# imazen/codec-eval

Hardware: AMD Instinct MI355X
Metric: metric MP/s (SSIMULACRA2+DSSIM+Butteraugli) at 1/2/4/8 GPU; HBM-roofline % (higher is better)
Workload: dtype f32

## Files before the change

### codec-eval_amd/__init__.py

```python
from __future__ import annotations

import ctypes as C
import os
from dataclasses import dataclass
from typing import Iterable, List, Optional, Sequence, Tuple

import numpy as np

os.environ.setdefault("GPU_MAX_HW_QUEUES", "16")

_HERE = os.path.dirname(os.path.abspath(__file__))
LIB_PATH = os.environ.get("CE_METRICS_LIB") or os.path.join(_HERE, "libce_metrics_hip.so")
INCLUDE_DIR = os.path.join(os.path.dirname(_HERE), "include")

CE_OK, CE_ERR_DIM_MISMATCH, CE_ERR_BAD_LENGTH, CE_ERR_TOO_SMALL, CE_ERR_BACKEND, CE_ERR_INVALID_ARG = range(6)
METRIC_DSSIM, METRIC_SSIMULACRA2, METRIC_BUTTERAUGLI, METRIC_PSNR = 1, 2, 4, 8
FLAG_XYB_ROUNDTRIP = 1
FLAG_BUTTERAUGLI_DIFFMAP = 1 << 1
FLAG_SSIMULACRA2_MAPS = 1 << 2
PIXEL_RGB8, PIXEL_RGBA8, PIXEL_RGB16_10BIT, PIXEL_RGBA16_10BIT = 0, 1, 2, 3
BATCH_REFERENCES, BATCH_TESTS = 0, 1
DEFAULT_INTENSITY_TARGET = 80.0
DSSIM_MAX_LEVELS = 5
SSIM2_MAX_SCALES = 6
# ... 678 lines not shown
        self.ctx._check(lib().ce_batch_set_test_lut(self._h, pair_index, ref_index, a.ctypes.data, a.nbytes, fmt, table._h if table else None))

    def bind_pair(self, pair_index: int, ref_index: int):
        self.ctx._check(lib().ce_batch_bind_pair(self._h, pair_index, ref_index))

    @property
    def reference_slab(self) -> int:
        return int(lib().ce_batch_reference_slab(self._h))

    @property
    def test_slab(self) -> int:
        return int(lib().ce_batch_test_slab(self._h))

    def run(self, n_pairs: int, config: MetricConfig, intensity_target: float = DEFAULT_INTENSITY_TARGET,
            butteraugli_diffmap: bool = False, ssimulacra2_maps: bool = False) -> List[CeScores]:
        out = (CeScores * n_pairs)()
        flags = config.flags | (FLAG_BUTTERAUGLI_DIFFMAP if butteraugli_diffmap else 0) | (FLAG_SSIMULACRA2_MAPS if ssimulacra2_maps else 0)
        self.ctx._check(lib().ce_batch_run(self._h, n_pairs, config.mask, flags, intensity_target, out))
        return list(out)

    def launch(self, n_pairs: int, config: MetricConfig, intensity_target: float = DEFAULT_INTENSITY_TARGET,
               butteraugli_diffmap: bool = False, ssimulacra2_maps: bool = False):
        flags = config.flags | (FLAG_BUTTERAUGLI_DIFFMAP if butteraugli_diffmap else 0) | (FLAG_SSIMULACRA2_MAPS if ssimulacra2_maps else 0)
        self.ctx._check(lib().ce_batch_launch(self._h, n_pairs, config.mask, flags, intensity_target))

    def collect(self, n_pairs: int) -> List[CeScores]:
        out = (CeScores * n_pairs)()
        self.ctx._check(lib().ce_batch_collect(self._h, n_pairs, out))
        return list(out)

    def butteraugli_pnorm3(self, n_pairs: int) -> np.ndarray:
        out = np.zeros(n_pairs, np.float64)
        self.ctx._check(lib().ce_batch_butteraugli_pnorm3(self._h, n_pairs, out.ctypes.data_as(_dp)))
        return out

    def butteraugli_diffmaps(self, first: int, count: int, block: int = 1) -> np.ndarray:
        return _read_diffmaps(self.ctx, lib().ce_batch_butteraugli_diffmap, self._h, self.width, self.height, first, count, block)

    def dssim_ssim_maps(self, level: int, first: int, count: int, block: int = 1):
        return _read_ssim_maps(self.ctx, lib().ce_batch_dssim_ssim_maps, self._h, self.width, self.height, level, first, count, block)

    def ssimulacra2_maps(self, scale: int, channel: int, kind: int, first: int, count: int, block: int = 1, maps: bool = True):
        return _read_ssim2_maps(self.ctx, lib().ce_batch_ssimulacra2_maps, self._h, self.width, self.height, scale, channel, kind,
                                first, count, block, maps)

    def image_heuristics(self, first: int, count: int, tests: bool = False) -> List[ImageHeuristics]:
        out = (CeImageHeuristics * max(count, 1))()
        self.ctx._check(lib().ce_batch_image_heuristics(self._h, BATCH_TESTS if tests else BATCH_REFERENCES, first, count, out))
        return [ImageHeuristics.from_c(out[i]) for i in range(count)]

    def debug_limit_scales(self, n: int):
        self.ctx._check(lib().ce_debug_ssim2_limit_scales(self._h, n))

    def debug_planes(self, scale: int, which: int, channel: int = 0) -> np.ndarray:
        nplanes = 5 if which == 4 else 3
        buf = np.empty(nplanes * self.width * self.height, np.float32)
        w, h = C.c_uint32(), C.c_uint32()
        self.ctx._check(lib().ce_debug_ssim2_planes(self._h, scale, which, channel, buf.ctypes.data, buf.size,
                                                     C.byref(w), C.byref(h)))
        return buf[: nplanes * w.value * h.value].reshape(nplanes, h.value, w.value).copy()

    def debug_dssim_walk_rows(self, rows: int):
        self.ctx._check(lib().ce_debug_dssim_walk_rows(self._h, rows))

    def debug_averages(self, pair_index: int) -> np.ndarray:
        avg = np.zeros((6, 3, 6), np.float64)
        ns = C.c_int()
        self.ctx._check(lib().ce_debug_ssim2_averages(self._h, pair_index, avg.ctypes.data_as(_dp), C.byref(ns)))
        return avg[: ns.value].copy()


class ReferenceHandle:

    def __init__(self, ctx: Context, reference, width: int, height: int, xyb_roundtrip: bool = False,
                 butteraugli_diffmap: bool = False, ssimulacra2_maps: bool = False):
        self.ctx, self.width, self.height = ctx, width, height
        r = _buf(reference)
        self._h = C.c_void_p()
        flags = ((FLAG_XYB_ROUNDTRIP if xyb_roundtrip else 0) | (FLAG_BUTTERAUGLI_DIFFMAP if butteraugli_diffmap else 0) |
                 (FLAG_SSIMULACRA2_MAPS if ssimulacra2_maps else 0))
        ctx._check(lib().ce_ref_create(ctx._h, r.ctypes.data, r.size, width, height, flags, C.byref(self._h)))

    def compare(self, test, config: MetricConfig = None, intensity_target: float = DEFAULT_INTENSITY_TARGET) -> MetricResult:
        config = config or MetricConfig.ssimulacra2_only()
        t = _buf(test)
        s = CeScores()
        self.ctx._check(lib().ce_ref_compare(self._h, t.ctypes.data, t.size, config.mask, intensity_target, C.byref(s)))
        return MetricResult.from_c(s)

    def compare_many(self, tests, config: MetricConfig = None, intensity_target: float = DEFAULT_INTENSITY_TARGET):
        config = config or MetricConfig.ssimulacra2_only()
        bufs = [_buf(t) for t in tests]
        n = len(bufs)
        if n == 0:
            return []
        ptrs = (C.c_void_p * n)(*[b.ctypes.data for b in bufs])
        lens = (_sz * n)(*[b.size for b in bufs])
        out = (CeScores * n)()
        self.ctx._check(lib().ce_ref_compare_many(self._h, ptrs, lens, n, config.mask, intensity_target, out))
        res = []
        for s in out:
            res.append(MetricResult.from_c(s) if s.status == 0 else _error_obj(s.status, self.ctx._err()))
        return res

    def butteraugli_diffmaps(self, first: int, count: int, block: int = 1) -> np.ndarray:
        return _read_diffmaps(self.ctx, lib().ce_ref_butteraugli_diffmap, self._h, self.width, self.height, first, count, block)

    def dssim_ssim_maps(self, level: int, first: int, count: int, block: int = 1):
# ... 104 lines not shown
```

### codec-eval_amd/csrc/ce_api.cpp

```cpp
#include <algorithm>
#include <atomic>
#include <condition_variable>
#include <functional>
#include <mutex>
#include <thread>
#include <cmath>
#include <cstdlib>
#include <cstring>
#include <new>

#include "ce_internal.h"

namespace {

thread_local std::string g_err_noctx;

int fail(ce_ctx *ctx, int code, const std::string &msg)
{
    if (ctx) ctx->err = msg; else g_err_noctx = msg;
    return code;
}

int bad_length(ce_ctx *ctx, size_t want, size_t got)
{
// ... 1595 lines not shown
    ctx->prof_filter = substring ? substring : "";
    return CE_OK;
}

int ce_prof_reset(ce_ctx *ctx)
{
    if (!ctx) return CE_ERR_INVALID_ARG;
    prof_drain(ctx);
    ctx->stats.clear();
    return CE_OK;
}

int ce_prof_count(ce_ctx *ctx)
{
    if (!ctx) return 0;
    prof_drain(ctx);
    return (int)ctx->stats.size();
}

int ce_prof_get(ce_ctx *ctx, int index, const char **name, uint64_t *launches, double *total_ms)
{
    if (!ctx || index < 0 || index >= (int)ctx->stats.size()) return CE_ERR_INVALID_ARG;
    prof_drain(ctx);
    if (name) *name = ctx->stats[index].name.c_str();
    if (launches) *launches = ctx->stats[index].launches;
    if (total_ms) *total_ms = ctx->stats[index].total_ms;
    return CE_OK;
}

int ce_timer_start(ce_ctx *ctx)
{
    if (!ctx) return CE_ERR_INVALID_ARG;
    CE_HIP(ctx, hipSetDevice(ctx->device));
    CE_HIP(ctx, hipEventRecord(ctx->t0, ctx->stream));
    return CE_OK;
}

int ce_timer_stop(ce_ctx *ctx, double *elapsed_ms)
{
    if (!ctx || !elapsed_ms) return CE_ERR_INVALID_ARG;
    CE_HIP(ctx, hipSetDevice(ctx->device));
    CE_HIP(ctx, hipEventRecord(ctx->t1, ctx->stream));
    CE_HIP(ctx, hipEventSynchronize(ctx->t1));
    float ms = 0.f;
    CE_HIP(ctx, hipEventElapsedTime(&ms, ctx->t0, ctx->t1));
    *elapsed_ms = ms;
    return CE_OK;
}


int ce_debug_ssim2_planes(ce_batch *b, int scale, int which, int channel, float *out, size_t out_floats,
                          uint32_t *w_out, uint32_t *h_out)
{
    if (!b || !out || !b->ssim2_ready || scale < 0 || scale >= b->n_scales) return CE_ERR_INVALID_ARG;
    ce_ctx *ctx = b->ctx;
    const ce_scale_dims &d = b->sd[scale];
    const int nplanes = which == 4 ? CE_SSIM2_STREAMS : 3;
    if (out_floats < (size_t)nplanes * d.w * d.h) return CE_ERR_INVALID_ARG;
    const uint32_t ref_slot = b->h_pair_ref[0], test_slot = b->max_refs;
    const float *src = nullptr;
    switch (which) {
        case 0:
        case 1:
            if (scale == 0) return CE_ERR_INVALID_ARG;
            src = b->d_lin[scale] + (size_t)(which == 0 ? ref_slot : test_slot) * 3 * d.plane;
            break;
        case 2: src = b->d_xyb[scale] + (size_t)ref_slot * 3 * d.plane; break;
        case 3: src = b->d_xyb[scale] + (size_t)test_slot * 3 * d.plane; break;
        case 4:
            if (channel < 0 || channel > 2) return CE_ERR_INVALID_ARG;
            src = b->d_hbuf[scale] + (size_t)channel * CE_SSIM2_STREAMS * d.hplane;
            break;
        default: return CE_ERR_INVALID_ARG;
    }
    CE_HIP(ctx, hipSetDevice(ctx->device));
    CE_HIP(ctx, hipStreamSynchronize(ctx->stream));
    const size_t spl = which == 4 ? d.hplane : d.plane, spitch = which == 4 ? d.hpitch : d.pitch;
    for (int p = 0; p < nplanes; p++)
        CE_HIP(ctx, hipMemcpy2D(out + (size_t)p * d.w * d.h, (size_t)d.w * sizeof(float), src + (size_t)p * spl,
                                spitch * sizeof(float), (size_t)d.w * sizeof(float), d.h, hipMemcpyDeviceToHost));
    if (w_out) *w_out = d.w;
    if (h_out) *h_out = d.h;
    return CE_OK;
}

int ce_debug_ssim2_limit_scales(ce_batch *b, int max_scales)
{
    if (!b || max_scales < 1 || max_scales > CE_MAX_SCALES) return CE_ERR_INVALID_ARG;
    b->debug_max_scales = max_scales;
    return CE_OK;
}

int ce_debug_dssim_walk_rows(ce_batch *b, uint32_t rows)
{
    if (!b || (rows != 0 && (rows < 2 || rows > 64 || (rows & (rows - 1)) != 0))) return CE_ERR_INVALID_ARG;
    b->debug_ds_rows = rows;
    return CE_OK;
}

int ce_debug_ssim2_averages(ce_batch *b, uint32_t pair_index, double *avg, int *n_scales)
{
    if (!b || !avg || !b->ssim2_ready || pair_index >= b->max_pairs) return CE_ERR_INVALID_ARG;
    ce_ctx *ctx = b->ctx;
    CE_HIP(ctx, hipSetDevice(ctx->device));
    CE_HIP(ctx, hipStreamSynchronize(ctx->stream));
    CE_HIP(ctx, hipMemcpy(avg, b->d_avg + (size_t)pair_index * CE_MAX_SCALES * 18, sizeof(double) * CE_MAX_SCALES * 18,
                          hipMemcpyDeviceToHost));
    if (n_scales) *n_scales = b->n_scales;
    return CE_OK;
}

int ce_debug_ssim2_occupancy(int which) { return ce_ssim2_occupancy(which); }

int ce_debug_div_sweep(ce_ctx *ctx, uint64_t seed, uint64_t count, uint64_t *mismatches)
{
    if (!ctx || count == 0) return CE_ERR_INVALID_ARG;
    CE_HIP(ctx, hipSetDevice(ctx->device));
    return ce_butteraugli_div_sweep(ctx, seed, count, mismatches);
}

int ce_debug_calibrate_traffic(ce_ctx *ctx, size_t bytes)
{
    if (!ctx) return CE_ERR_INVALID_ARG;
    CE_HIP(ctx, hipSetDevice(ctx->device));
// ... 12 lines not shown
```

### codec-eval_amd/csrc/ce_plan.h

```cpp
#pragma once

#include <algorithm>
#include <cstdint>
#include <map>
#include <vector>

inline constexpr uint32_t ce_plan_ring_slots = 3;
inline constexpr size_t ce_plan_none = ~(size_t)0;

struct ce_plan_inputs {
    size_t budget;
    size_t per_pair;
    uint32_t pooled_pairs;
    size_t forced_chunks;
    size_t ramp;
};

struct ce_plan_chunk {
    uint32_t slot;
    uint32_t max_pairs;
    size_t collect_first;
    std::vector<std::vector<size_t>> refs;
};

inline void ce_plan_bucket(const std::vector<size_t> &items, const std::vector<const void *> &refs, const ce_plan_inputs &in,
                           uint32_t &ring, std::vector<ce_plan_chunk> &plan)
{
    std::map<const void *, size_t> group_of;
    std::vector<std::vector<size_t>> groups;
    for (size_t j = 0; j < items.size(); j++) {
        const size_t g = group_of.emplace(refs[j], groups.size()).first->second;
        if (g == groups.size()) groups.emplace_back();
        groups[g].push_back(items[j]);
    }
    const size_t n = items.size();
    const size_t n_chunks = in.forced_chunks ? std::min<size_t>(in.forced_chunks, std::max<size_t>(1, n))
                                             : std::min<size_t>(ce_plan_ring_slots, std::max<size_t>(1, n / 64));
    size_t target = std::min((n + n_chunks - 1) / n_chunks, std::max<size_t>(1, in.budget / std::max<size_t>(in.per_pair, 1)));
    if (in.pooled_pairs < target && (size_t)in.pooled_pairs * 4 >= target * 3) target = in.pooled_pairs;
    std::vector<std::vector<size_t>> split;
    for (auto &g : groups)
        for (size_t o = 0; o < g.size(); o += target) split.emplace_back(g.begin() + o, g.begin() + std::min(g.size(), o + target));
    const bool several = n > target;
    size_t limit = (several && in.ramp && ring == 0) ? std::min(in.ramp, target) : target;
    const size_t bucket_begin = plan.size();
    for (size_t g0 = 0, g1 = 0; g0 < split.size(); g0 = g1) {
        size_t count = 0;
        while (g1 < split.size() && (count == 0 || count + split[g1].size() <= limit)) count += split[g1++].size();
        limit = std::min(target, limit * 2);
        ce_plan_chunk c{ring++ % ce_plan_ring_slots, (uint32_t)(several ? std::max(count, target) : count), ce_plan_none,
                        std::vector<std::vector<size_t>>(split.begin() + g0, split.begin() + g1)};
        for (size_t p = bucket_begin; p < plan.size(); p++)
            if (plan[p].slot == c.slot) c.collect_first = p;
        plan.push_back(std::move(c));
    }
}

struct ce_plan_entry {
    uint32_t tile, pair;
};

struct ce_xcd_keys {
    uint32_t channels;
    uint32_t keys_per_channel;
    uint32_t tiles_per_key;
    uint32_t round_to = 1;
};

inline bool operator==(const ce_xcd_keys &a, const ce_xcd_keys &b)
{
    return a.channels == b.channels && a.keys_per_channel == b.keys_per_channel && a.tiles_per_key == b.tiles_per_key &&
           a.round_to == b.round_to;
}

inline std::vector<ce_plan_entry> ce_plan_xcd_list(const uint32_t *pair_ref, uint32_t n_pairs, uint32_t n_refs, const ce_xcd_keys &k)
{
    std::vector<std::vector<uint32_t>> pairs_of(n_refs);
    for (uint32_t p = 0; p < n_pairs; p++) pairs_of[pair_ref[p]].push_back(p);
    std::vector<ce_plan_entry> cls[8];
    uint32_t key = 0;
    for (const auto &pairs : pairs_of) {
        if (pairs.empty()) continue;
        for (uint32_t c = 0; c < k.channels; c++)
            for (uint32_t j = 0; j < k.keys_per_channel; j++, key++)
                for (uint32_t sub = 0; sub < k.tiles_per_key; sub++)
                    for (uint32_t p : pairs) cls[key & 7].push_back({(j * k.tiles_per_key + sub) | c << 16, p});
    }
    size_t len = 0;
    for (const auto &v : cls) len = std::max(len, v.size());
    len = (len + k.round_to - 1) / k.round_to * k.round_to;
    std::vector<ce_plan_entry> list(len * 8, ce_plan_entry{~0u, 0u});
    for (uint32_t x = 0; x < 8; x++)
        for (size_t i = 0; i < cls[x].size(); i++) list[i * 8 + x] = cls[x][i];
    return list;
}

inline uint32_t ce_plan_dssim_levels(uint32_t w, uint32_t h, uint32_t max_levels, uint32_t *level_w, uint32_t *level_h)
{
    if (w == 0 || h == 0) return 0;
    uint32_t n = 0;
    while (n < max_levels) {
        level_w[n] = w;
        level_h[n] = h;
        n++;
        if (w < 8 || h < 8) break;
        w /= 2;
        h /= 2;
    }
    return n;
}

inline uint32_t ce_plan_ssim2_scales(uint32_t w, uint32_t h, uint32_t max_scales, uint32_t *scale_w, uint32_t *scale_h)
{
    uint32_t n = 0;
    for (uint32_t s = 0; s < max_scales; s++) {
        if (w < 8 || h < 8) break;
        if (s > 0) {
            w = w / 2 + (w & 1);
            h = h / 2 + (h & 1);
        }
        scale_w[n] = w;
        scale_h[n] = h;
        n++;
    }
    return n;
}
```

### codec-eval_amd/csrc/ssim2.hip

```cpp
#include <algorithm>
#include <cstdlib>

#include "ce_internal.h"

namespace {

struct rg_consts {
    float mul_in[3];
    float mul_prev[3];
};

constexpr int kColsPerBlock = 64;

constexpr int kTailLevels = CE_MAX_SCALES - 1;
struct lvl_table {
    uint32_t n, first_level;
    uint32_t blk_end[kTailLevels];
    uint32_t w[kTailLevels], h[kTailLevels], pitch[kTailLevels];
    size_t plane[kTailLevels];
    const float *xyb[kTailLevels];
    float *hbuf[kTailLevels];
};

__device__ __forceinline__ uint32_t slot_of(uint32_t z, uint32_t n_refs_used, uint32_t max_refs)
// ... 124 lines not shown
            }
            sum[0] += r;
            sum[1] += g;
            sum[2] += bl;
            linear_to_xyb_positive(r, g, bl, cbrt_bias, X[dx], Y[dx], B[dx]);
        }
        if (yr < h) {
            const size_t o = (size_t)y * pitch + 2 * qx;
            if (2 * qx + 1 < w) {
                *reinterpret_cast<float2 *>(xo + o) = make_float2(X[0], X[1]);
                *reinterpret_cast<float2 *>(xo + o + plane) = make_float2(Y[0], Y[1]);
                *reinterpret_cast<float2 *>(xo + o + 2 * plane) = make_float2(B[0], B[1]);
            } else {
                xo[o] = X[0];
                xo[o + plane] = Y[0];
                xo[o + 2 * plane] = B[0];
            }
        }
    }
    if (has_next) {
        float *lo = lin_out + (size_t)slot * 3 * oplane + (size_t)qy * opitch + qx;
        lo[0] = sum[0] * 0.25f;
        lo[oplane] = sum[1] * 0.25f;
        lo[2 * oplane] = sum[2] * 0.25f;
    }
}

__device__ __forceinline__ float rg_step(float sum, float (&prev)[3], float (&prev2)[3], const rg_consts &rg)
{
    float o[3];
#pragma unroll
    for (int k = 0; k < 3; k++) {
        float v = sum * rg.mul_in[k];
        v = __builtin_fmaf(-1.0f, prev2[k], v);
        prev2[k] = prev[k];
        v = __builtin_fmaf(rg.mul_prev[k], prev[k], v);
        prev[k] = v;
        o[k] = v;
    }
    return o[0] + o[1] + o[2];
}

__device__ __forceinline__ void lds_barrier()
{
    asm volatile("" ::: "memory");
    __builtin_amdgcn_s_waitcnt(0xC07F);
    __builtin_amdgcn_s_barrier();
    asm volatile("" ::: "memory");
}

#ifndef CE_HB_ROWS
#define CE_HB_ROWS 32
#endif
constexpr int HB_ROWS = CE_HB_ROWS, HB_CW = 32, HB_LD = HB_ROWS + 1, HB_THREADS = 256;
constexpr int HB_LOADS = 2 * HB_ROWS * 8;
constexpr int HB_LSLOTS = (HB_LOADS + 63) / 64;
static_assert(HB_ROWS * CE_SSIM2_STREAMS <= HB_THREADS, "one task per thread");
constexpr int HB_HALF = HB_CW * HB_LD;
constexpr int HB_STORES = CE_SSIM2_STREAMS * HB_ROWS * (HB_CW / 4);

typedef float hb_f2 __attribute__((ext_vector_type(2)));

struct hblur_state {
    hb_f2 p01, q01;
    float p2, q2;
    float d[10];
};

__device__ __forceinline__ void hblur_chunk(const float *__restrict__ p_cur, const float *__restrict__ q_cur, bool plain,
                                            float *__restrict__ so, hblur_state &st, const rg_consts &rg)
{
    const hb_f2 n01 = {rg.mul_in[0], rg.mul_in[1]}, d01 = {rg.mul_prev[0], rg.mul_prev[1]};
#pragma unroll
    for (int half = 0; half < 2; half++) {
        float in[HB_CW / 2];
#pragma unroll
        for (int i = 0; i < HB_CW / 2; i++) in[i] = p_cur[(half * (HB_CW / 2) + i) * HB_LD];
#pragma unroll
        for (int i = 0; i < HB_CW / 2; i++) {
            const float q = q_cur[(half * (HB_CW / 2) + i) * HB_LD];
            in[i] = in[i] * (plain ? 1.0f : q);
        }
#pragma unroll
        for (int i = 0; i < HB_CW / 2; i++) {
            const int e = half * (HB_CW / 2) + i;
            const float sum = st.d[e % 10] + in[i];
            st.d[e % 10] = in[i];
            hb_f2 v01 = hb_f2{sum, sum} * n01;
            v01 = v01 - st.q01;
            st.q01 = st.p01;
            v01 = __builtin_elementwise_fma(d01, st.p01, v01);
            st.p01 = v01;
            float v2 = sum * rg.mul_in[2];
            v2 = v2 - st.q2;
            st.q2 = st.p2;
            v2 = __builtin_fmaf(rg.mul_prev[2], st.p2, v2);
            st.p2 = v2;
            so[e * HB_LD] = v01.x + v01.y + v2;
        }
    }
    float t[10];
#pragma unroll
    for (int j = 0; j < 10; j++) t[j] = st.d[(j + HB_CW) % 10];
#pragma unroll
    for (int j = 0; j < 10; j++) st.d[j] = t[j];
}

template <int LEVEL>
__global__ __launch_bounds__(HB_THREADS) void k_ssim2_hblur_lds(const float *__restrict__ xyb,
                                                                const uint32_t *__restrict__ pair_ref,
                                                                float *__restrict__ hbuf, uint32_t w, uint32_t h,
                                                                uint32_t pitch, size_t plane, uint32_t max_refs,
                                                                rg_consts rg, lvl_table tab, const uint2 *__restrict__ work,
                                                                const uint32_t *__restrict__ pair_first)
{
    __shared__ float s_in[2][2 * HB_HALF];
    __shared__ float s_out[CE_SSIM2_STREAMS * HB_HALF];
    const uint32_t tid = threadIdx.x, lane = tid & 63, wv = tid >> 6;
    uint32_t bx = blockIdx.x, c = blockIdx.y, p = blockIdx.z;
    if (work) {
        const uint2 wi = work[blockIdx.x];
        if (wi.x == ~0u) return;
        bx = wi.x & 0xffffu, c = wi.x >> 16, p = wi.y;
    }
    if (LEVEL < 0) {
        uint32_t l = 0;
        while (l + 1 < tab.n && bx >= tab.blk_end[l]) l++;
        bx -= l ? tab.blk_end[l - 1] : 0;
        xyb = tab.xyb[l], hbuf = tab.hbuf[l];
        w = tab.w[l], h = tab.h[l], pitch = tab.pitch[l], plane = tab.plane[l];
    }
    const uint32_t y0 = bx * HB_ROWS;
    const float *ga = xyb + ((size_t)pair_ref[p] * 3 + c) * plane;
    const float *gb = xyb + ((size_t)(max_refs + p) * 3 + c) * plane;
    const int n_chunks = (int)(pitch / HB_CW);
    const bool loader = wv == 3;
    const float *l_src[HB_LSLOTS];
    uint32_t l_dst[HB_LSLOTS];
    uint32_t l_row[HB_LSLOTS];
    const uint32_t lq = lane & 7;
#pragma unroll
    for (int m = 0; m < HB_LSLOTS; m++) {
        const uint32_t j = min(64u * m + lane, (uint32_t)HB_LOADS - 1), pl = j / (HB_ROWS * 8), row = (j % (HB_ROWS * 8)) >> 3;
        l_row[m] = 64u * m + lane < (uint32_t)HB_LOADS ? y0 + row : ~0u;
        l_src[m] = (pl ? gb : ga) + (size_t)min(y0 + row, h - 1) * pitch;
        l_dst[m] = pl * (2 * HB_HALF) + (4 * lq) * HB_LD + row;
    }
    float4 pf[HB_LSLOTS];
    auto load_chunk = [&](int k) {
        if (loader) {
            const int col = max(HB_CW * k - 28 + 4 * (int)lq, 0);
#pragma unroll
            for (int m = 0; m < HB_LSLOTS; m++) pf[m] = *reinterpret_cast<const float4 *>(l_src[m] + col);
        }
    };
    auto stash_chunk = [&](int k) {
        if (loader) {
            const int col = HB_CW * k - 28 + 4 * (int)lq;
            float *base = &s_in[0][0] + (k & 1) * HB_HALF;
#pragma unroll
            for (int m = 0; m < HB_LSLOTS; m++) {
                if (l_row[m] == ~0u) continue;
                float *dst = base + l_dst[m];
                const bool rv = l_row[m] < h && col >= 0;
                dst[0] = (rv && col < (int)w) ? pf[m].x : 0.0f;
                dst[HB_LD] = (rv && col + 1 < (int)w) ? pf[m].y : 0.0f;
                dst[2 * HB_LD] = (rv && col + 2 < (int)w) ? pf[m].z : 0.0f;
                dst[3 * HB_LD] = (rv && col + 3 < (int)w) ? pf[m].w : 0.0f;
            }
        }
    };

    load_chunk(0);
    stash_chunk(0);
    if (n_chunks > 1) load_chunk(1);
    __syncthreads();

    const bool full = pair_first[p] == p;
    const uint32_t n_jobs = full ? CE_SSIM2_STREAMS : 3;
    const bool worker = tid < n_jobs * HB_ROWS;
    const uint32_t tj = worker ? tid / HB_ROWS : 0, tr = worker ? tid % HB_ROWS : 0;
    const uint32_t ts = full ? tj : (tj == 0 ? 1u : tj + 2u);
    const bool plain = ts < 2;
    const float *sp = &s_in[(ts == 1 || ts == 3) ? 1 : 0][tr];
    const float *sq = &s_in[(ts == 2) ? 0 : 1][tr];
    float *so = &s_out[ts * HB_HALF + tr];
    hblur_state st;
    st.p01 = st.q01 = hb_f2{0.0f, 0.0f};
    st.p2 = st.q2 = 0.0f;
#pragma unroll
    for (int j = 0; j < 10; j++) st.d[j] = 0.0f;
    float *obase = hbuf + ((size_t)p * 3 + c) * CE_SSIM2_STREAMS * plane;

    for (int k = 0; k < n_chunks; k++) {
        if (k + 1 < n_chunks) stash_chunk(k + 1);
        if (k + 2 < n_chunks) load_chunk(k + 2);
        const uint32_t oc = (k & 1) * HB_HALF;
        if (worker) hblur_chunk(sp + oc, sq + oc, plain, so, st, rg);
        lds_barrier();
        if (k > 0 && !loader) {
#pragma unroll
            for (int it = 0; it < (HB_STORES + 191) / 192; it++) {
                const uint32_t idx = it * 192 + tid;
                if (idx >= n_jobs * (HB_ROWS * 8)) break;
                const uint32_t oj = idx / (HB_ROWS * 8), rem = idx % (HB_ROWS * 8), orow = rem >> 3, oq = rem & 7;
                const uint32_t os = full ? oj : (oj == 0 ? 1u : oj + 2u);
                const float *src = &s_out[os * HB_HALF + (4 * oq) * HB_LD + orow];
                const float4 v = make_float4(src[0], src[HB_LD], src[2 * HB_LD], src[3 * HB_LD]);
                if (y0 + orow < h)
                    *reinterpret_cast<float4 *>(obase + (size_t)os * plane + (size_t)(y0 + orow) * pitch + HB_CW * (k - 1) + 4 * oq) = v;
            }
        }
        lds_barrier();
    }
}

__device__ __forceinline__ double wave_sum(double v)
{
#pragma unroll
    for (int off = 32; off > 0; off >>= 1) v += __shfl_down(v, off, 64);
    return v;
}

constexpr int VB_G = 4;
constexpr int VB_PLANES = 7;
constexpr int VB_SLOT = VB_G * 64;
constexpr int VB_GROUP = VB_PLANES * VB_SLOT;

struct vblur_state {
    float prev[CE_SSIM2_STREAMS][3], prev2[CE_SSIM2_STREAMS][3];
    float rr[16][CE_SSIM2_STREAMS];
    double acc[6];
};

template <int GG, bool CHECKED, bool STORE>
__device__ __forceinline__ void vblur_group(vblur_state &st, const float *__restrict__ slot, int g, uint32_t h,
                                            const rg_consts &rg, float *__restrict__ map, uint32_t pitch, size_t plane,
                                            uint32_t lane, bool active)
{
    const float C2 = 0.0009f;
    float gacc[6] = {0.f, 0.f, 0.f, 0.f, 0.f, 0.f};
#pragma unroll
    for (int e = 0; e < VB_G; e++) {
        const uint32_t i = (uint32_t)(4 * g + e);
        constexpr int base = 4 * GG;
        const int re = base + e;
        float v[CE_SSIM2_STREAMS];
#pragma unroll
        for (int s = 0; s < CE_SSIM2_STREAMS; s++) {
            const float ld = slot[s * VB_SLOT + e * 64];
            const float right = (!CHECKED || i < h) ? ld : 0.0f;
            const float left = st.rr[(re + 6) & 15][s];
            st.rr[re][s] = right;
            v[s] = rg_step(left + right, st.prev[s], st.prev2[s], rg);
        }
        if (!CHECKED || (i >= 4 && i < h + 4)) {
            const float img1 = slot[5 * VB_SLOT + e * 64], img2 = slot[6 * VB_SLOT + e * 64];
            const float mu1 = v[0], mu2 = v[1], s11 = v[2], s22 = v[3], s12 = v[4];
            const float mu11 = mu1 * mu1, mu22 = mu2 * mu2, mu12 = mu1 * mu2;
            const float mu_diff = mu1 - mu2;
            const float num_m = __builtin_fmaf(mu_diff, -mu_diff, 1.0f);
            const float num_s = __builtin_fmaf(2.0f, s12 - mu12, C2);
            const float denom_s = (s11 - mu11) + (s22 - mu22) + C2;
// ... 231 lines not shown
    for (ce_xcd_list *L : {&b->work_h, &b->work_v, &b->work_ht, &b->work_vt}) ce_free_xcd_list(L);
    b->ssim2_ready = false;
}

static int ssim2_allocate(ce_batch *b)
{
    ce_ctx *ctx = b->ctx;
    const int ns = b->n_scales;
    const size_t slots = (size_t)b->max_refs + b->max_pairs;
    for (int s = 1; s < ns; s++)
        CE_HIP(ctx, hipMalloc(&b->d_lin[s], slots * 3 * b->sd[s].plane * sizeof(float)));
    for (int s = 0; s < ns; s++) {
        CE_HIP(ctx, hipMalloc(&b->d_xyb[s], slots * 3 * b->sd[s].plane * sizeof(float)));
        CE_HIP(ctx, hipMalloc(&b->d_hbuf[s], (size_t)b->max_pairs * 3 * CE_SSIM2_STREAMS * b->sd[s].plane * sizeof(float)));
        if (s == 0 && !(b->lvl_stream[0] = ce_ctx_aux_stream(ctx, ce_ctx::AUX_SSIM2_L0))) return CE_ERR_BACKEND;
        CE_HIP(ctx, hipEventCreateWithFlags(&b->ev_prep[s], hipEventDisableTiming));
        CE_HIP(ctx, hipEventCreateWithFlags(&b->ev_done[s], hipEventDisableTiming));
    }
    b->max_vblocks = (b->sd[0].w + kColsPerBlock - 1) / kColsPerBlock;
    CE_HIP(ctx, hipMalloc(&b->d_partials, (size_t)b->max_pairs * CE_MAX_SCALES * 3 * b->max_vblocks * 6 * sizeof(double)));
    CE_HIP(ctx, hipMalloc(&b->d_avg, (size_t)b->max_pairs * CE_MAX_SCALES * 18 * sizeof(double)));
    return CE_OK;
}

int ce_ssim2_prepare(ce_batch *b)
{
    if (b->ssim2_ready) return CE_OK;
    uint32_t sw[CE_MAX_SCALES], sh[CE_MAX_SCALES];
    const int ns = (int)ce_plan_ssim2_scales(b->w, b->h, CE_MAX_SCALES, sw, sh);
    for (int s = 0; s < ns; s++) {
        const uint32_t w = sw[s], h = sh[s];
        ce_scale_dims &d = b->sd[s];
        d.w = w;
        d.h = h;
        d.pitch = ((w + HB_CW - 1) / HB_CW) * HB_CW + HB_CW;
        d.plane = (size_t)d.pitch * (((size_t)h + HB_ROWS - 1) / HB_ROWS * HB_ROWS);
        d.hpitch = d.pitch;
        d.hplane = d.plane;
    }
    b->n_scales = ns;
    if (ns == 0) return CE_OK;
    const int rc = ssim2_allocate(b);
    if (rc != CE_OK) {
        const std::string why = b->ctx->err;
        ce_ssim2_free(b);
        (void)hipGetLastError();
        b->ctx->err = why;
        return rc;
    }
    b->ssim2_ready = true;
    return CE_OK;
}

static int build_pass_list(ce_batch *b, uint32_t n_pairs, uint32_t n_blocks, ce_xcd_list *L)
{
    if (n_blocks > 0xffffu) {
        b->ctx->err = "SSIMULACRA2: image too large for the block index of the work list";
        return CE_ERR_INVALID_ARG;
    }
    return ce_build_xcd_list(b, n_pairs, ce_xcd_keys{3, n_blocks, 1}, L);
}

int ce_launch_ssim2(ce_batch *b, const uint8_t *d_refs, uint32_t n_refs_used, uint32_t n_pairs, bool store_maps)
{
    ce_ctx *ctx = b->ctx;
    int rc = ce_ssim2_prepare(b);
    if (rc != CE_OK) return rc;
    ssim2_map_table maps{};
    if (store_maps) {
        if (!b->s2_map) {
            size_t total = 0;
            for (int s = 0; s < b->n_scales; s++) total += (size_t)b->max_pairs * 9 * b->sd[s].plane;
            if (hipMalloc(&b->s2_map, total * sizeof(float)) != hipSuccess) {
                b->s2_map = nullptr;
                (void)hipGetLastError();
                ctx->err = "out of device memory for the SSIMULACRA2 maps";
                return CE_ERR_BACKEND;
            }
            size_t off = 0;
            for (int s = 0; s < b->n_scales; s++) {
                b->s2_map_lvl[s] = b->s2_map + off;
                off += (size_t)b->max_pairs * 9 * b->sd[s].plane;
            }
        }
        for (int s = 0; s < b->n_scales; s++) maps.lvl[s] = b->s2_map_lvl[s];
    }
    rg_consts rg;
    ce_ssim2_recursive_gaussian(rg.mul_in, rg.mul_prev);
    const uint32_t n_slots = n_refs_used + n_pairs;
    const bool cached = b->keep_ref_pyramid && b->ssim2_ref_src == d_refs && b->ssim2_ref_count >= n_refs_used &&
                        b->ssim2_ref_levels == std::min(b->n_scales, b->debug_max_scales);
    const uint32_t z0 = cached ? n_refs_used : 0;
    if (!cached) b->ref_builds[0]++;
    using hblur_fn = void (*)(const float *, const uint32_t *, float *, uint32_t, uint32_t, uint32_t, size_t, uint32_t,
                              rg_consts, lvl_table, const uint2 *, const uint32_t *);
    using vblur_fn = void (*)(const float *, const float *, const uint32_t *, double *, uint32_t, uint32_t, uint32_t,
                              size_t, uint32_t, uint32_t, uint32_t, rg_consts, lvl_table, const uint2 *, const uint32_t *,
                              ssim2_map_table);
    const hblur_fn h_l0 = k_ssim2_hblur_lds<0>, h_tail = k_ssim2_hblur_lds<-1>;
    const vblur_fn v_l0 = k_ssim2_vblur_dma<0, false>, v_tail = k_ssim2_vblur_dma<-1, false>;
    const vblur_fn v_l0_map = k_ssim2_vblur_dma<0, true>, v_tail_map = k_ssim2_vblur_dma<-1, true>;
    scale_geom g{};
    const int levels = std::min(b->n_scales, b->debug_max_scales);
    hipStream_t s0 = ctx->prof_serial ? CE_STREAM(ctx) : b->lvl_stream[0];
    hipStream_t s1 = CE_STREAM(ctx);
    lvl_table tab{};
    lvl_table tab_v{};
    for (int s = 0; s < levels; s++) {
        const ce_scale_dims &d = b->sd[s];
        const bool has_next = s + 1 < levels;
        const ce_scale_dims &nd = b->sd[has_next ? s + 1 : s];
        const dim3 quad_grid(((d.w + 1) / 2 + 63) / 64, ((d.h + 1) / 2 + 3) / 4, n_slots - z0);
        if (s == 0)
            CE_LAUNCH(ctx, "ssim2_prep_u8", k_ssim2_prep<true>, quad_grid, dim3(256), 0, d_refs, b->d_tests, ctx->d_lut_ssim2,
                      (const float *)nullptr, b->d_xyb[0], b->d_lin[1], d.w, d.h, d.pitch, d.plane, nd.pitch, nd.plane,
                      has_next ? 1 : 0, b->img_bytes, n_refs_used, b->max_refs, z0);
        else
            CE_LAUNCH(ctx, "ssim2_prep", k_ssim2_prep<false>, quad_grid, dim3(256), 0, d_refs, b->d_tests, ctx->d_lut_ssim2,
                      (const float *)b->d_lin[s], b->d_xyb[s], b->d_lin[has_next ? s + 1 : s], d.w, d.h, d.pitch, d.plane,
                      nd.pitch, nd.plane, has_next ? 1 : 0, b->img_bytes, n_refs_used, b->max_refs, z0);
        const uint32_t hblk = (d.h + HB_ROWS - 1) / HB_ROWS, vblk = (d.w + kColsPerBlock - 1) / kColsPerBlock;
        g.npix[s] = d.w * d.h;
        g.nblk[s] = vblk;
        if (s == 0) {
            if (s0 != CE_STREAM(ctx)) {
                CE_HIP(ctx, hipEventRecord(b->ev_prep[0], CE_STREAM(ctx)));
                CE_HIP(ctx, hipStreamWaitEvent(s0, b->ev_prep[0], 0));
            }
            if ((rc = build_pass_list(b, n_pairs, hblk, &b->work_h)) != CE_OK) return rc;
            if ((rc = build_pass_list(b, n_pairs, vblk, &b->work_v)) != CE_OK) return rc;
            CE_LAUNCH_ON(ctx, s0, "ssim2_hblur_L0", h_l0, dim3(b->work_h.len), dim3(HB_THREADS), 0, b->d_xyb[0], b->d_pair_ref,
                         b->d_hbuf[0], d.w, d.h, d.pitch, d.plane, b->max_refs, rg, tab, (const uint2 *)b->work_h.d,
                         (const uint32_t *)b->d_pair_first);
#define CE_VBLUR_L0_ARGS                                                                                                   \
    b->d_hbuf[0], b->d_xyb[0], b->d_pair_ref, b->d_partials, d.w, d.h, d.pitch, d.plane, b->max_refs, 0u, b->max_vblocks, rg, tab, \
        (const uint2 *)b->work_v.d, (const uint32_t *)b->d_pair_first, maps
            if (store_maps)
                CE_LAUNCH_ON(ctx, s0, "ssim2_vblur_ssim_map_L0", v_l0_map, dim3(b->work_v.len), dim3(64), 0, CE_VBLUR_L0_ARGS);
            else
                CE_LAUNCH_ON(ctx, s0, "ssim2_vblur_ssim_L0", v_l0, dim3(b->work_v.len), dim3(64), 0, CE_VBLUR_L0_ARGS);
#undef CE_VBLUR_L0_ARGS
            if (s0 != CE_STREAM(ctx)) CE_HIP(ctx, hipEventRecord(b->ev_done[0], s0));
        } else {
            const uint32_t l = tab.n++;
            tab_v.n = tab.n;
            tab.first_level = tab_v.first_level = 1;
            tab.blk_end[l] = (l ? tab.blk_end[l - 1] : 0) + hblk;
            tab_v.blk_end[l] = (l ? tab_v.blk_end[l - 1] : 0) + vblk;
            tab.w[l] = tab_v.w[l] = d.w;
            tab.h[l] = tab_v.h[l] = d.h;
            tab.pitch[l] = tab_v.pitch[l] = d.pitch;
            tab.plane[l] = tab_v.plane[l] = d.plane;
            tab.xyb[l] = tab_v.xyb[l] = b->d_xyb[s];
            tab.hbuf[l] = tab_v.hbuf[l] = b->d_hbuf[s];
        }
    }
    if (tab.n) {
        if (s1 != CE_STREAM(ctx)) {
            CE_HIP(ctx, hipEventRecord(b->ev_prep[1], CE_STREAM(ctx)));
            CE_HIP(ctx, hipStreamWaitEvent(s1, b->ev_prep[1], 0));
        }
        if ((rc = build_pass_list(b, n_pairs, tab.blk_end[tab.n - 1], &b->work_ht)) != CE_OK) return rc;
        if ((rc = build_pass_list(b, n_pairs, tab_v.blk_end[tab_v.n - 1], &b->work_vt)) != CE_OK) return rc;
        CE_LAUNCH_ON(ctx, s1, "ssim2_hblur_L1-5", h_tail, dim3(b->work_ht.len), dim3(HB_THREADS), 0,
                     (const float *)nullptr, b->d_pair_ref, (float *)nullptr, 0u, 0u, 0u, (size_t)0, b->max_refs, rg, tab,
                     (const uint2 *)b->work_ht.d, (const uint32_t *)b->d_pair_first);
#define CE_VBLUR_TAIL_ARGS                                                                                                  \
    (const float *)nullptr, (const float *)nullptr, b->d_pair_ref, b->d_partials, 0u, 0u, 0u, (size_t)0, b->max_refs, 0u,        \
        b->max_vblocks, rg, tab_v, (const uint2 *)b->work_vt.d, (const uint32_t *)b->d_pair_first, maps
        if (store_maps)
            CE_LAUNCH_ON(ctx, s1, "ssim2_vblur_ssim_map_L1-5", v_tail_map, dim3(b->work_vt.len), dim3(64), 0, CE_VBLUR_TAIL_ARGS);
        else
            CE_LAUNCH_ON(ctx, s1, "ssim2_vblur_ssim_L1-5", v_tail, dim3(b->work_vt.len), dim3(64), 0, CE_VBLUR_TAIL_ARGS);
#undef CE_VBLUR_TAIL_ARGS
        if (s1 != CE_STREAM(ctx)) CE_HIP(ctx, hipEventRecord(b->ev_done[1], s1));
    }
    if (s0 != CE_STREAM(ctx)) {
        CE_HIP(ctx, hipStreamWaitEvent(CE_STREAM(ctx), b->ev_done[0], 0));
        if (tab.n && s1 != CE_STREAM(ctx)) CE_HIP(ctx, hipStreamWaitEvent(CE_STREAM(ctx), b->ev_done[1], 0));
    }
    if (b->keep_ref_pyramid && !cached) {
        b->ssim2_ref_src = d_refs;
        b->ssim2_ref_count = n_refs_used;
        b->ssim2_ref_levels = levels;
    }
    CE_LAUNCH(ctx, "ssim2_finalize", k_ssim2_finalize, dim3(n_pairs), dim3(128), 0, b->d_partials, b->d_avg,
              b->d_scores, (uint32_t)levels, b->max_vblocks, g);
    CE_HIP(ctx, hipGetLastError());
    return CE_OK;
}

int ce_ssim2_cbrt_sweep(ce_ctx *ctx, uint32_t first_bits, uint64_t count, uint64_t *mismatches, uint64_t *slow_path)
{
    unsigned long long *d = nullptr, h[2] = {0, 0};
    CE_HIP(ctx, hipMalloc(&d, sizeof(h)));
    CE_HIP(ctx, hipMemsetAsync(d, 0, sizeof(h), ctx->stream));
    CE_LAUNCH(ctx, "cbrt_sweep", k_cbrt_sweep, dim3(4096), dim3(256), 0, first_bits, count, d);
    CE_HIP(ctx, hipMemcpyAsync(h, d, sizeof(h), hipMemcpyDeviceToHost, ctx->stream));
    CE_HIP(ctx, hipStreamSynchronize(ctx->stream));
    CE_HIP(ctx, hipFree(d));
    if (mismatches) *mismatches = h[0];
    if (slow_path) *slow_path = h[1];
    return CE_OK;
}

int ce_ssim2_read_maps(ce_batch *b, uint32_t scale, uint32_t channel, uint32_t kind, uint32_t first, uint32_t count,
                       uint32_t block, float *maps, double *norms)
{
    ce_ctx *ctx = b->ctx;
    if (norms) {
        CE_HIP(ctx, hipMemcpy2DAsync(norms, 2 * sizeof(double), b->d_avg + (size_t)first * CE_MAX_SCALES * 18 + scale * 18 + channel * 6 + 2 * kind,
                                     CE_MAX_SCALES * 18 * sizeof(double), 2 * sizeof(double), count, hipMemcpyDeviceToHost, ctx->stream));
        if (!maps) CE_HIP(ctx, hipStreamSynchronize(ctx->stream));
    }
    if (!maps) return CE_OK;
    const ce_scale_dims &d = b->sd[scale];
    return ce_read_map_cells(b, "ssim2_block_max", b->s2_map_lvl[scale] + (size_t)(channel * 3 + kind) * d.plane,
                             ce_map_geom{d.w, d.h, d.pitch, 9 * d.plane}, first, count, block, false, &b->s2_cells, &b->s2_cells_cap,
                             maps);
// ... 12 lines not shown
```

Before: 18910.

## Group test images sharing a reference into one SSIMULACRA2 horizontal-blur block

The horizontal-blur kernel for SSIMULACRA2 can now process up to HB_T (default 2) test images that share the same reference in one block. The reference rows are loaded into LDS once and reused for each test's cross and squared products. The work list packs a group size and member index into each entry, and the kernel resolves group members through the reference offset and index tables. This cuts repeated reference-plane loads and the number of blocks. In exchange, each block uses more LDS for the extra input and output planes, which may lower occupancy, and the decode logic is more complex. A debug accessor gains a pair selector to inspect per-pair hblur buffers.

Result: no change. 19040, median of 6 (+0.7%).

```diff
diff --git a/codec-eval_amd/__init__.py b/codec-eval_amd/__init__.py
--- a/codec-eval_amd/__init__.py
+++ b/codec-eval_amd/__init__.py
@@ -754,8 +754,9 @@
     def debug_limit_scales(self, n: int):
         self.ctx._check(lib().ce_debug_ssim2_limit_scales(self._h, n))
 
-    def debug_planes(self, scale: int, which: int, channel: int = 0) -> np.ndarray:
+    def debug_planes(self, scale: int, which: int, channel: int = 0, pair: int = 0) -> np.ndarray:
         nplanes = 5 if which == 4 else 3
+        which |= pair << 8
         buf = np.empty(nplanes * self.width * self.height, np.float32)
         w, h = C.c_uint32(), C.c_uint32()
         self.ctx._check(lib().ce_debug_ssim2_planes(self._h, scale, which, channel, buf.ctypes.data, buf.size,
diff --git a/codec-eval_amd/csrc/ce_api.cpp b/codec-eval_amd/csrc/ce_api.cpp
--- a/codec-eval_amd/csrc/ce_api.cpp
+++ b/codec-eval_amd/csrc/ce_api.cpp
@@ -1671,7 +1671,10 @@
 int ce_debug_ssim2_planes(ce_batch *b, int scale, int which, int channel, float *out, size_t out_floats,
                           uint32_t *w_out, uint32_t *h_out)
 {
-    if (!b || !out || !b->ssim2_ready || scale < 0 || scale >= b->n_scales) return CE_ERR_INVALID_ARG;
+    if (!b || !out || !b->ssim2_ready || scale < 0 || scale >= b->n_scales || which < 0) return CE_ERR_INVALID_ARG;
+    const uint32_t pair = (uint32_t)which >> 8;
+    which &= 0xff;
+    if (pair && (which != 4 || pair >= b->max_pairs)) return CE_ERR_INVALID_ARG;
     ce_ctx *ctx = b->ctx;
     const ce_scale_dims &d = b->sd[scale];
     const int nplanes = which == 4 ? CE_SSIM2_STREAMS : 3;
@@ -1688,7 +1691,7 @@
         case 3: src = b->d_xyb[scale] + (size_t)test_slot * 3 * d.plane; break;
         case 4:
             if (channel < 0 || channel > 2) return CE_ERR_INVALID_ARG;
-            src = b->d_hbuf[scale] + (size_t)channel * CE_SSIM2_STREAMS * d.hplane;
+            src = b->d_hbuf[scale] + ((size_t)pair * 3 + channel) * CE_SSIM2_STREAMS * d.hplane;
             break;
         default: return CE_ERR_INVALID_ARG;
     }
diff --git a/codec-eval_amd/csrc/ce_plan.h b/codec-eval_amd/csrc/ce_plan.h
--- a/codec-eval_amd/csrc/ce_plan.h
+++ b/codec-eval_amd/csrc/ce_plan.h
@@ -65,13 +65,16 @@
     uint32_t keys_per_channel;
     uint32_t tiles_per_key;
     uint32_t round_to = 1;
+    uint32_t group = 1;
 };
 
 inline bool operator==(const ce_xcd_keys &a, const ce_xcd_keys &b)
 {
     return a.channels == b.channels && a.keys_per_channel == b.keys_per_channel && a.tiles_per_key == b.tiles_per_key &&
-           a.round_to == b.round_to;
+           a.round_to == b.round_to && a.group == b.group;
 }
+
+inline constexpr uint32_t ce_plan_group_shift = 18, ce_plan_group_index_shift = 20, ce_plan_group_index_max = 0xfffu;
 
 inline std::vector<ce_plan_entry> ce_plan_xcd_list(const uint32_t *pair_ref, uint32_t n_pairs, uint32_t n_refs, const ce_xcd_keys &k)
 {
@@ -83,8 +86,20 @@
         if (pairs.empty()) continue;
         for (uint32_t c = 0; c < k.channels; c++)
             for (uint32_t j = 0; j < k.keys_per_channel; j++, key++)
-                for (uint32_t sub = 0; sub < k.tiles_per_key; sub++)
-                    for (uint32_t p : pairs) cls[key & 7].push_back({(j * k.tiles_per_key + sub) | c << 16, p});
+                for (uint32_t sub = 0; sub < k.tiles_per_key; sub++) {
+                    const uint32_t tile = (j * k.tiles_per_key + sub) | c << 16;
+                    if (k.group <= 1) {
+                        for (uint32_t p : pairs) cls[key & 7].push_back({tile, p});
+                        continue;
+                    }
+                    cls[key & 7].push_back({tile, pairs[0]});
+                    for (size_t i = 1, n; i < pairs.size(); i += n) {
+                        n = std::min<size_t>(std::min(k.group, 4u), pairs.size() - i);
+                        if (i > ce_plan_group_index_max) n = 1;
+                        const uint32_t tag = n > 1 ? (uint32_t)(n - 1) << ce_plan_group_shift | (uint32_t)i << ce_plan_group_index_shift : 0;
+                        cls[key & 7].push_back({tile | tag, pairs[i]});
+                    }
+                }
     }
     size_t len = 0;
     for (const auto &v : cls) len = std::max(len, v.size());
diff --git a/codec-eval_amd/csrc/ssim2.hip b/codec-eval_amd/csrc/ssim2.hip
--- a/codec-eval_amd/csrc/ssim2.hip
+++ b/codec-eval_amd/csrc/ssim2.hip
@@ -200,12 +200,20 @@
 #ifndef CE_HB_ROWS
 #define CE_HB_ROWS 32
 #endif
+#ifndef CE_HB_T
+#define CE_HB_T 2
+#endif
 constexpr int HB_ROWS = CE_HB_ROWS, HB_CW = 32, HB_LD = HB_ROWS + 1, HB_THREADS = 256;
-constexpr int HB_LOADS = 2 * HB_ROWS * 8;
+constexpr int HB_T = CE_HB_T;
+constexpr int HB_PLANES = 1 + HB_T;
+constexpr int HB_JOBS = 3 * HB_T > CE_SSIM2_STREAMS ? 3 * HB_T : CE_SSIM2_STREAMS;
+constexpr int HB_WORKERS = HB_THREADS - 64;
+constexpr int HB_LOADS = HB_PLANES * HB_ROWS * 8;
 constexpr int HB_LSLOTS = (HB_LOADS + 63) / 64;
-static_assert(HB_ROWS * CE_SSIM2_STREAMS <= HB_THREADS, "one task per thread");
+static_assert(HB_T >= 1 && HB_T <= 4, "the work list's entry holds a group size of 1..4");
+static_assert(HB_ROWS * HB_JOBS <= HB_WORKERS, "one task per thread of the worker waves");
 constexpr int HB_HALF = HB_CW * HB_LD;
-constexpr int HB_STORES = CE_SSIM2_STREAMS * HB_ROWS * (HB_CW / 4);
+constexpr int HB_STORES = HB_JOBS * HB_ROWS * (HB_CW / 4);
 
 typedef float hb_f2 __attribute__((ext_vector_type(2)));
 
@@ -260,16 +268,28 @@
                                                                 float *__restrict__ hbuf, uint32_t w, uint32_t h,
                                                                 uint32_t pitch, size_t plane, uint32_t max_refs,
                                                                 rg_consts rg, lvl_table tab, const uint2 *__restrict__ work,
-                                                                const uint32_t *__restrict__ pair_first)
-{
-    __shared__ float s_in[2][2 * HB_HALF];
-    __shared__ float s_out[CE_SSIM2_STREAMS * HB_HALF];
+                                                                const uint32_t *__restrict__ pair_first,
+                                                                const uint32_t *__restrict__ ref_off,
+                                                                const uint32_t *__restrict__ ref_idx)
+{
+    __shared__ float s_in[HB_PLANES][2 * HB_HALF];
+    __shared__ float s_out[HB_JOBS * HB_HALF];
     const uint32_t tid = threadIdx.x, lane = tid & 63, wv = tid >> 6;
-    uint32_t bx = blockIdx.x, c = blockIdx.y, p = blockIdx.z;
+    uint32_t bx = blockIdx.x, c = blockIdx.y, p = blockIdx.z, n_t = 1, gi = 0;
     if (work) {
         const uint2 wi = work[blockIdx.x];
         if (wi.x == ~0u) return;
-        bx = wi.x & 0xffffu, c = wi.x >> 16, p = wi.y;
+        bx = wi.x & 0xffffu, c = (wi.x >> 16) & 3u, p = wi.y;
+        n_t = min(1u + ((wi.x >> ce_plan_group_shift) & 3u), (uint32_t)HB_T), gi = wi.x >> ce_plan_group_index_shift;
+    }
+    uint32_t pt[HB_T];
+#pragma unroll
+    for (int t = 0; t < HB_T; t++) pt[t] = p;
+    if (n_t > 1) {
+        const uint32_t *members = ref_idx + ref_off[pair_ref[p]] + gi;
+#pragma unroll
+        for (int t = 1; t < HB_T; t++)
+            if ((uint32_t)t < n_t) pt[t] = members[t];
     }
     if (LEVEL < 0) {
         uint32_t l = 0;
@@ -280,8 +300,8 @@
     }
     const uint32_t y0 = bx * HB_ROWS;
     const float *ga = xyb + ((size_t)pair_ref[p] * 3 + c) * plane;
-    const float *gb = xyb + ((size_t)(max_refs + p) * 3 + c) * plane;
     const int n_chunks = (int)(pitch / HB_CW);
+    const uint32_t n_loads = (1 + n_t) * (HB_ROWS * 8);
     const bool loader = wv == 3;
     const float *l_src[HB_LSLOTS];
     uint32_t l_dst[HB_LSLOTS];
@@ -289,17 +309,22 @@
     const uint32_t lq = lane & 7;
 #pragma unroll
     for (int m = 0; m < HB_LSLOTS; m++) {
-        const uint32_t j = min(64u * m + lane, (uint32_t)HB_LOADS - 1), pl = j / (HB_ROWS * 8), row = (j % (HB_ROWS * 8)) >> 3;
-        l_row[m] = 64u * m + lane < (uint32_t)HB_LOADS ? y0 + row : ~0u;
+        const uint32_t j = min(64u * m + lane, n_loads - 1), pl = j / (HB_ROWS * 8), row = (j % (HB_ROWS * 8)) >> 3;
+        uint32_t lp = pt[0];
+#pragma unroll
+        for (int t = 1; t < HB_T; t++) lp = pl == (uint32_t)(1 + t) ? pt[t] : lp;
+        const float *gb = xyb + ((size_t)(max_refs + lp) * 3 + c) * plane;
+        l_row[m] = 64u * m + lane < n_loads ? y0 + row : ~0u;
         l_src[m] = (pl ? gb : ga) + (size_t)min(y0 + row, h - 1) * pitch;
         l_dst[m] = pl * (2 * HB_HALF) + (4 * lq) * HB_LD + row;
     }
-    float4 pf[HB_LSLOTS];
+    float4 pf[HB_LSLOTS] = {};
     auto load_chunk = [&](int k) {
         if (loader) {
             const int col = max(HB_CW * k - 28 + 4 * (int)lq, 0);
 #pragma unroll
-            for (int m = 0; m < HB_LSLOTS; m++) pf[m] = *reinterpret_cast<const float4 *>(l_src[m] + col);
+            for (int m = 0; m < HB_LSLOTS; m++)
+                if (l_row[m] != ~0u) pf[m] = *reinterpret_cast<const float4 *>(l_src[m] + col);
         }
     };
     auto stash_chunk = [&](int k) {
@@ -325,20 +350,21 @@
     __syncthreads();
 
     const bool full = pair_first[p] == p;
-    const uint32_t n_jobs = full ? CE_SSIM2_STREAMS : 3;
+    const uint32_t n_jobs = full ? CE_SSIM2_STREAMS : 3 * n_t;
     const bool worker = tid < n_jobs * HB_ROWS;
     const uint32_t tj = worker ? tid / HB_ROWS : 0, tr = worker ? tid % HB_ROWS : 0;
-    const uint32_t ts = full ? tj : (tj == 0 ? 1u : tj + 2u);
+    const uint32_t tk = tj % 3;
+    const uint32_t ts = full ? tj : (tk == 0 ? 1u : tk + 2u);
+    const uint32_t tb = full ? 1u : 1u + tj / 3;
     const bool plain = ts < 2;
-    const float *sp = &s_in[(ts == 1 || ts == 3) ? 1 : 0][tr];
-    const float *sq = &s_in[(ts == 2) ? 0 : 1][tr];
-    float *so = &s_out[ts * HB_HALF + tr];
+    const float *sp = &s_in[(ts == 1 || ts == 3) ? tb : 0][tr];
+    const float *sq = &s_in[(ts == 2) ? 0 : tb][tr];
+    float *so = &s_out[tj * HB_HALF + tr];
     hblur_state st;
     st.p01 = st.q01 = hb_f2{0.0f, 0.0f};
     st.p2 = st.q2 = 0.0f;
 #pragma unroll
     for (int j = 0; j < 10; j++) st.d[j] = 0.0f;
-    float *obase = hbuf + ((size_t)p * 3 + c) * CE_SSIM2_STREAMS * plane;
 
     for (int k = 0; k < n_chunks; k++) {
         if (k + 1 < n_chunks) stash_chunk(k + 1);
@@ -348,15 +374,19 @@
         lds_barrier();
         if (k > 0 && !loader) {
 #pragma unroll
-            for (int it = 0; it < (HB_STORES + 191) / 192; it++) {
-                const uint32_t idx = it * 192 + tid;
+            for (int it = 0; it < (HB_STORES + HB_WORKERS - 1) / HB_WORKERS; it++) {
+                const uint32_t idx = it * HB_WORKERS + tid;
                 if (idx >= n_jobs * (HB_ROWS * 8)) break;
                 const uint32_t oj = idx / (HB_ROWS * 8), rem = idx % (HB_ROWS * 8), orow = rem >> 3, oq = rem & 7;
-                const uint32_t os = full ? oj : (oj == 0 ? 1u : oj + 2u);
-                const float *src = &s_out[os * HB_HALF + (4 * oq) * HB_LD + orow];
+                const uint32_t ok = oj % 3, os = full ? oj : (ok == 0 ? 1u : ok + 2u), ot = full ? 0u : oj / 3;
+                uint32_t op = pt[0];
+#pragma unroll
+                for (int t = 1; t < HB_T; t++) op = ot == (uint32_t)t ? pt[t] : op;
+                const float *src = &s_out[oj * HB_HALF + (4 * oq) * HB_LD + orow];
                 const float4 v = make_float4(src[0], src[HB_LD], src[2 * HB_LD], src[3 * HB_LD]);
                 if (y0 + orow < h)
-                    *reinterpret_cast<float4 *>(obase + (size_t)os * plane + (size_t)(y0 + orow) * pitch + HB_CW * (k - 1) + 4 * oq) = v;
+                    *reinterpret_cast<float4 *>(hbuf + (((size_t)op * 3 + c) * CE_SSIM2_STREAMS + os) * plane +
+                                                (size_t)(y0 + orow) * pitch + HB_CW * (k - 1) + 4 * oq) = v;
             }
         }
         lds_barrier();
@@ -694,13 +724,13 @@
     return CE_OK;
 }
 
-static int build_pass_list(ce_batch *b, uint32_t n_pairs, uint32_t n_blocks, ce_xcd_list *L)
+static int build_pass_list(ce_batch *b, uint32_t n_pairs, uint32_t n_blocks, ce_xcd_list *L, uint32_t group = 1)
 {
     if (n_blocks > 0xffffu) {
         b->ctx->err = "SSIMULACRA2: image too large for the block index of the work list";
         return CE_ERR_INVALID_ARG;
     }
-    return ce_build_xcd_list(b, n_pairs, ce_xcd_keys{3, n_blocks, 1}, L);
+    return ce_build_xcd_list(b, n_pairs, ce_xcd_keys{3, n_blocks, 1, 1, group}, L);
 }
 
 int ce_launch_ssim2(ce_batch *b, const uint8_t *d_refs, uint32_t n_refs_used, uint32_t n_pairs, bool store_maps)
@@ -735,7 +765,7 @@
     const uint32_t z0 = cached ? n_refs_used : 0;
     if (!cached) b->ref_builds[0]++;
     using hblur_fn = void (*)(const float *, const uint32_t *, float *, uint32_t, uint32_t, uint32_t, size_t, uint32_t,
-                              rg_consts, lvl_table, const uint2 *, const uint32_t *);
+                              rg_consts, lvl_table, const uint2 *, const uint32_t *, const uint32_t *, const uint32_t *);
     using vblur_fn = void (*)(const float *, const float *, const uint32_t *, double *, uint32_t, uint32_t, uint32_t,
                               size_t, uint32_t, uint32_t, uint32_t, rg_consts, lvl_table, const uint2 *, const uint32_t *,
                               ssim2_map_table);
@@ -769,11 +799,11 @@
                 CE_HIP(ctx, hipEventRecord(b->ev_prep[0], CE_STREAM(ctx)));
                 CE_HIP(ctx, hipStreamWaitEvent(s0, b->ev_prep[0], 0));
             }
-            if ((rc = build_pass_list(b, n_pairs, hblk, &b->work_h)) != CE_OK) return rc;
+            if ((rc = build_pass_list(b, n_pairs, hblk, &b->work_h, HB_T)) != CE_OK) return rc;
             if ((rc = build_pass_list(b, n_pairs, vblk, &b->work_v)) != CE_OK) return rc;
             CE_LAUNCH_ON(ctx, s0, "ssim2_hblur_L0", h_l0, dim3(b->work_h.len), dim3(HB_THREADS), 0, b->d_xyb[0], b->d_pair_ref,
                          b->d_hbuf[0], d.w, d.h, d.pitch, d.plane, b->max_refs, rg, tab, (const uint2 *)b->work_h.d,
-                         (const uint32_t *)b->d_pair_first);
+                         (const uint32_t *)b->d_pair_first, (const uint32_t *)b->d_ref_off, (const uint32_t *)b->d_ref_idx);
 #define CE_VBLUR_L0_ARGS                                                                                                   \
     b->d_hbuf[0], b->d_xyb[0], b->d_pair_ref, b->d_partials, d.w, d.h, d.pitch, d.plane, b->max_refs, 0u, b->max_vblocks, rg, tab, \
         (const uint2 *)b->work_v.d, (const uint32_t *)b->d_pair_first, maps
@@ -802,11 +832,12 @@
             CE_HIP(ctx, hipEventRecord(b->ev_prep[1], CE_STREAM(ctx)));
             CE_HIP(ctx, hipStreamWaitEvent(s1, b->ev_prep[1], 0));
         }
-        if ((rc = build_pass_list(b, n_pairs, tab.blk_end[tab.n - 1], &b->work_ht)) != CE_OK) return rc;
+        if ((rc = build_pass_list(b, n_pairs, tab.blk_end[tab.n - 1], &b->work_ht, HB_T)) != CE_OK) return rc;
         if ((rc = build_pass_list(b, n_pairs, tab_v.blk_end[tab_v.n - 1], &b->work_vt)) != CE_OK) return rc;
         CE_LAUNCH_ON(ctx, s1, "ssim2_hblur_L1-5", h_tail, dim3(b->work_ht.len), dim3(HB_THREADS), 0,
                      (const float *)nullptr, b->d_pair_ref, (float *)nullptr, 0u, 0u, 0u, (size_t)0, b->max_refs, rg, tab,
-                     (const uint2 *)b->work_ht.d, (const uint32_t *)b->d_pair_first);
+                     (const uint2 *)b->work_ht.d, (const uint32_t *)b->d_pair_first, (const uint32_t *)b->d_ref_off,
+                     (const uint32_t *)b->d_ref_idx);
 #define CE_VBLUR_TAIL_ARGS                                                                                                  \
     (const float *)nullptr, (const float *)nullptr, b->d_pair_ref, b->d_partials, 0u, 0u, 0u, (size_t)0, b->max_refs, 0u,        \
         b->max_vblocks, rg, tab_v, (const uint2 *)b->work_vt.d, (const uint32_t *)b->d_pair_first, maps
```
